# langtech-bsc/quantool

Hardware: AMD Instinct MI355X
Metric: quantized weights/sec (GPTQ int4, Llama-3-8B, 512 calib samples) (higher is better)
Workload: dtype f32

## Files before the change

### include/quantool_amd.h

```cpp
#ifndef QUANTOOL_AMD_H
#define QUANTOOL_AMD_H

#include <stddef.h>
#include <stdint.h>

#ifdef __cplusplus
extern "C" {
#endif

typedef void* qt_stream_t;

enum qt_status {
    QT_OK = 0,
    QT_ERR_INVALID = -1,
    QT_ERR_NOT_PD = -2,
    QT_ERR_WORKSPACE = -3,
    QT_ERR_HIP = -4,
    QT_ERR_UNSUPPORTED = -5
};

enum qt_dtype { QT_F32 = 0, QT_BF16 = 1, QT_F16 = 2 };

int qt_version(void);
const char* qt_last_error(void);
// ... 37 lines not shown
                             const uint8_t* dead, int group_size, int symmetric, int num_bits, float* W_f32, float* scale,
                             float* zp, float* scale_t, float* zp_t, int64_t ld_t, qt_stream_t stream);

size_t qt_gptq_sweep_workspace_bytes(int R, int K, int blocksize);
int qt_gptq_sweep(float* W, int R, int K, const float* U, const float* scale_t, const float* zp_t,
                  int G, const int32_t* g_idx, int blocksize, int num_bits, int8_t* Qt,
                  float* loss, void* workspace, size_t workspace_bytes, qt_stream_t stream);

int qt_gptq_sweep_grouped(float* W, int R, int K, const float* U, int64_t strideU, int n_groups, const int32_t* row_end,
                          const float* scale_t, const float* zp_t, int G, const int32_t* g_idx, int blocksize,
                          int num_bits, int8_t* Qt, float* loss, void* workspace, size_t workspace_bytes,
                          qt_stream_t stream);

int qt_pack_int4(const int8_t* Qt, int R, int K, const int32_t* col_src, int32_t* packed,
                 qt_stream_t stream);

int qt_dequantize(const int8_t* Qt, int R, int K, const int32_t* col_src, const float* scale,
                  const float* zp, int G, const int32_t* g_of_col, void* out, int out_dtype,
                  int64_t ldo, qt_stream_t stream);

size_t qt_awq_weight_mean_workspace_bytes(int R, int K);
int qt_awq_weight_mean_accumulate(const void* W, int w_dtype, int R, int K, int64_t ldw, int group_size,
                                  float* w_sum, void* workspace, size_t workspace_bytes,
                                  qt_stream_t stream);
int qt_awq_scales(const float* x_abs_sum, int64_t n_tokens, const float* w_sum, int64_t n_rows, int K,
                  int n_grid, int duo_scaling, float* scales, qt_stream_t stream);
int qt_symmetrize_lower(float* G, int K, qt_stream_t stream);
size_t qt_awq_loss_workspace_bytes(int R, int K);
int qt_awq_loss(const void* W, int w_dtype, int R, int K, int64_t ldw, const float* s, int group_size,
                int symmetric, int num_bits, const float* Gfull, int64_t n_tokens, int exact, float weight,
                int accumulate, float* loss_out, void* workspace, size_t workspace_bytes, qt_stream_t stream);
size_t qt_awq_losses_workspace_bytes(int R, int K, int n_grid);
int qt_awq_losses(const void* W, int w_dtype, int R, int K, int64_t ldw, const float* scales, int n_grid,
                  int group_size, int symmetric, int num_bits, const float* Gfull, int64_t n_tokens, float weight,
                  int accumulate, float* losses, void* workspace, size_t workspace_bytes, qt_stream_t stream);
int qt_argmin_f32(const float* values, int n, int32_t* index_out, qt_stream_t stream);
int qt_awq_pseudo_quantize(const void* W, int w_dtype, int R, int K, int64_t ldw, const float* s, int group_size,
                           int symmetric, int num_bits, void* out, int64_t ldo, qt_stream_t stream);
int qt_scale_columns(const void* W, int w_dtype, int R, int K, int64_t ldw, const float* s, int divide,
                     void* out, int64_t ldo, qt_stream_t stream);
int qt_rtn_quantize(const void* W, int w_dtype, int R, int K, int64_t ldw, const float* scale,
                    const float* zp, int G, int group_size, int num_bits, int8_t* Qt, qt_stream_t stream);

size_t qt_col_absmax_workspace_bytes(int R, int K);
int qt_col_absmax_accumulate(const void* W, int w_dtype, int R, int K, int64_t ldw, float* wmax,
                             void* workspace, size_t workspace_bytes, qt_stream_t stream);
int qt_smoothquant_scales(const float* cmin, const float* cmax, const float* wmax, int K, float alpha,
                          float* s, qt_stream_t stream);

size_t qt_sgemm_tn_f32_workspace_bytes(int M, int N);
int qt_sgemm_tn_f32(const float* A, int64_t lda, const float* B, int64_t ldb, const float* Cin,
                    int64_t ldcin, float* Cout, int64_t ldcout, int M, int N, int kdim, int skip_zero_k,
                    int mode, int allow_split_k, void* workspace, size_t workspace_bytes, qt_stream_t stream);

int qt_xtx_tile_table_check(int K, int* n_tiles_out, int* chunk_panels_out, int* round_panels_out);

size_t qt_xtx_dot_workspace_bytes(int64_t n_tokens, int K);
int qt_xtx_dot(const void* X, int x_dtype, int64_t n_tokens, int K, int64_t ldx, const float* H, double scale,
               float* out, int accumulate, void* workspace, size_t workspace_bytes, qt_stream_t stream);

size_t qt_gemm3_tn_f32_workspace_bytes(int M, int N, int k);
int qt_gemm3_tn_f32(const float* A, int64_t lda, const float* B, int64_t ldb, float* C, int64_t ldc, int M,
                    int N, int k, int kind, void* workspace, size_t workspace_bytes, qt_stream_t stream);
int qt_gemm3_tn_f32_ex(const float* A, int64_t lda, const float* B, int64_t ldb, float* C, int64_t ldc, int M, int N,
                       int k, int kind, int tri, int tight, int batch, int64_t bsA, int64_t bsB, int64_t bsC,
                       void* workspace, size_t workspace_bytes, qt_stream_t stream);

int qt_gemm3_plan_check(int Tm, int Tn, int c_end, int tri, int* n_items_out, int* n_slabs_out, int* longest_out);
#define QT_I8_MID_MAX_M 128
#define QT_I8_MID_K_UNIT 128
#define QT_I8_RING_K_UNIT 128
#define QT_I8_RING_SLOTS 8
#define QT_I8_RING_LEAD 6
#define QT_I8_RING_W4_K_UNIT 128
#define QT_I8_RING_W4_SLOTS 8
#define QT_I8_RING_W4_LEAD 6
enum qt_weight_format { QT_W_INT8 = 0, QT_W_INT4_PACKED = 1 };
int qt_quantize_tokens_i8(const void* X, int x_dtype, int64_t M, int K, int64_t ldx, const int32_t* col_perm,
                          int symmetric, int8_t* Xq, float* s_x, int32_t* zp_x, qt_stream_t stream);
int qt_gemm_i8(const int8_t* Xq, int64_t M, int K, const void* Wq, int w_format, int N, const float* s_x,
               const int32_t* zp_x, const float* s_w, int G, const int32_t* wsum, const void* bias, void* Y,
               int out_dtype, int64_t ldy, qt_stream_t stream);
int qt_gemm_i8_skinny(const int8_t* Xq, int M, int K, const void* Wq, int w_format, int N, const float* s_x,
                      const int32_t* zp_x, const float* s_w, int G, const int32_t* wsum, const void* bias, void* Y,
                      int out_dtype, int64_t ldy, qt_stream_t stream);
int qt_gemm_i8_ring(const int8_t* Xq, int64_t M, int K, const void* Wq, int w_format, int N, const float* s_x,
                    const int32_t* zp_x, const float* s_w, int G, const int32_t* wsum, const void* bias, void* Y,
                    int out_dtype, int64_t ldy, qt_stream_t stream);
int qt_gemm_i8_ring_w4(const int8_t* Xq, int64_t M, int K, const void* Wq, int w_format, int N, const float* s_x,
                       const int32_t* zp_x, const float* s_w, int G, const int32_t* wsum, const void* bias, void* Y,
                       int out_dtype, int64_t ldy, qt_stream_t stream);
int qt_gemm_i8_mid(const int8_t* Xq, int64_t M, int K, const void* Wq, int w_format, int N, const float* s_x,
                   const int32_t* zp_x, const float* s_w, int G, const int32_t* wsum, const void* bias, void* Y,
                   int out_dtype, int64_t ldy, qt_stream_t stream);

int qt_moe_route(const void* top_k_index, int index_is_int64, int64_t T, int k, int E, int32_t* offsets,
                 int32_t* src_token, int32_t* src_slot, int32_t* row_of, qt_stream_t stream);
int qt_gemm_i8_grouped(const int8_t* Xq, int K, const int32_t* row_idx, int64_t R, const int32_t* offsets, int E,
                       const void* Wq, int w_format, int N, const float* s_x, const int32_t* zp_x, const float* s_w,
                       int G, const int32_t* wsum, void* Y, int out_dtype, int64_t ldy, qt_stream_t stream);
int qt_gemm_i8_skinny_grouped(const int8_t* Xq, int K, const int32_t* row_idx, int64_t R, const int32_t* offsets,
                              int E, const void* Wq, int w_format, int N, const float* s_x, const int32_t* zp_x,
                              const float* s_w, int G, const int32_t* wsum, void* Y, int out_dtype, int64_t ldy,
                              qt_stream_t stream);
int qt_gemm_i8_ring_grouped(const int8_t* Xq, int K, const int32_t* row_idx, int64_t R, const int32_t* offsets, int E,
                            const void* Wq, int w_format, int N, const float* s_x, const int32_t* zp_x,
// ... 24 lines not shown
```

### quantool_amd/csrc/cholesky.hip

```cpp
#include <stdlib.h>
#include <string.h>

#include <map>
#include <tuple>
#include <vector>

#include "common.h"
#include "gemm3_tn.h"
#include "sgemm_tn.h"

namespace {

constexpr int NB = 128;
constexpr int NBO_MAX = 1024;
static int chol_block_env(const char* name) {
    const char* e = getenv(name);
    if (!e) return 0;
    int x = atoi(e) / 128 * 128;
    return x < 128 ? 128 : (x > NBO_MAX ? NBO_MAX : x);
}
struct G3Step {
    int n_items = 0, n_red = 0;
    size_t item_off = 0, red_off = 0;
};
// ... 464 lines not shown
        }
}

__global__ __launch_bounds__(256) void transpose_lower_block_kernel(const float* __restrict__ Y, int64_t ldy, int w,
                                                                    float* __restrict__ XT, int ldx, int64_t bsY,
                                                                    int64_t bsXT) {
    if (blockIdx.z) {
        Y += (size_t)blockIdx.z * bsY;
        XT += (size_t)blockIdx.z * bsXT;
    }
    __shared__ float tile[32][33];
    const int bx = blockIdx.x * 32, by = blockIdx.y * 32;
    const int tx = threadIdx.x & 31, ty = threadIdx.x >> 5;
    for (int r = ty; r < 32; r += 8) {
        const int m = bx + r, k = by + tx;
        tile[r][tx] = (m < w && k < w && k <= m) ? Y[(size_t)m * ldy + k] : 0.0f;
    }
    __syncthreads();
    for (int r = ty; r < 32; r += 8) {
        const int k = by + r, m = bx + tx;
        if (k < w && m < w) XT[(size_t)k * ldx + m] = tile[tx][r];
    }
}

__global__ __launch_bounds__(256) void flat_reverse_lower_to_upper_kernel(float* __restrict__ U, int K, int64_t bsU) {
    U += (size_t)blockIdx.z * bsU;
    const int j = blockIdx.x * blockDim.x + threadIdx.x;
    const int i = blockIdx.y;
    if (j >= K || j < i) return;
    const size_t e = (size_t)i * K + j;
    const size_t pe = (size_t)(K - 1 - i) * K + (K - 1 - j);
    if (i == j) {
        if (e <= pe) {
            const float t = U[e];
            U[e] = U[pe];
            U[pe] = t;
        }
    } else {
        U[e] = U[pe];
        U[pe] = 0.0f;
    }
}

__global__ __launch_bounds__(256) void identity_if_failed_kernel(float* __restrict__ U, int K,
                                                                 const int32_t* __restrict__ info, int64_t bsU) {
    if (info[blockIdx.z] == 0) return;
    U += (size_t)blockIdx.z * bsU;
    for (int i = blockIdx.x; i < K; i += gridDim.x)
        for (int j = threadIdx.x; j < K; j += blockDim.x) U[(size_t)i * K + j] = (i == j) ? 1.0f : 0.0f;
}

}

static size_t chol_problem_ws_bytes(int K, const CholG3Plan* g3) {
    const size_t nb = (K + NB - 1) / NB;
    const size_t split = (size_t)2048 * NB * NB * 4 + (size_t)NBO_MAX * K * 4;
    size_t n = (size_t)NB * K * 4 + (size_t)NBO_MAX * K * 4 + (size_t)NBO_MAX * NBO_MAX * 4 + nb * (NB * NB + RD_STRIDE) * 4 + split + 256;
    if (g3->any) n += 2 * qt_align_up((size_t)3 * K * K * 2, 256) + (size_t)g3->max_slabs * 256 * 256 * 4 + 256;
    return qt_align_up(n, 256);
}

extern "C" size_t qt_cholesky_inverse_upper_batched_workspace_bytes(int K, int n_problems) {
    if (K <= 0 || n_problems <= 0) return 0;
    int nbo_, nbi_;
    const CholG3Plan* g3 = chol_blocks(K, nbo_, nbi_);
    return (size_t)n_problems * chol_problem_ws_bytes(K, g3) + g3->blob_bytes + 512;
}

extern "C" size_t qt_cholesky_inverse_upper_workspace_bytes(int K) {
    return qt_cholesky_inverse_upper_batched_workspace_bytes(K, 1);
}

static int chol_run(float* A, int64_t strideA, int K, float* U, int64_t strideU, int32_t* info, int nprob, void* workspace,
                    size_t workspace_bytes, hipStream_t stream) {
    const size_t need = qt_cholesky_inverse_upper_batched_workspace_bytes(K, nprob);
    if (!workspace || workspace_bytes < need) {
        qt_set_error("qt_cholesky_inverse_upper: workspace %zu < required %zu", workspace_bytes, need);
        return QT_ERR_WORKSPACE;
    }
    const int nblk = (K + NB - 1) / NB;
    char* ws = (char*)qt_align_up((size_t)workspace, 256);
    int NBO, NBI;
    const CholG3Plan* g3 = chol_blocks(K, NBO, NBI);
    const size_t prob_bytes = chol_problem_ws_bytes(K, g3);
    const int64_t sW = (int64_t)(prob_bytes / 4);
    const int64_t sA = nprob > 1 ? strideA : 0, sU = nprob > 1 ? strideU : 0;
    float* T = (float*)ws;
    float* TI = T + (size_t)NB * K;
    float* XT = TI + (size_t)NBO_MAX * K;
    float* Rd = XT + (size_t)NBO_MAX * NBO_MAX;
    float* Dinv = Rd + (size_t)nblk * RD_STRIDE;
    float* split_ws = Dinv + (size_t)nblk * NB * NB;
    const size_t split_ws_bytes = (size_t)2048 * NB * NB * 4 + (size_t)NBO_MAX * K * 4;
    unsigned short *Rpl = nullptr, *Ypl = nullptr;
    float* g3_slabs = nullptr;
    char* g3_tab = nullptr;
    const int64_t plane_stride = (int64_t)K * K;
    if (g3->any) {
        char* q = (char*)qt_align_up((size_t)((char*)split_ws + split_ws_bytes), 256);
        Rpl = (unsigned short*)q;
        q += qt_align_up((size_t)3 * K * K * 2, 256);
        Ypl = (unsigned short*)q;
        q += qt_align_up((size_t)3 * K * K * 2, 256);
        g3_slabs = (float*)q;
        g3_tab = (char*)qt_align_up((size_t)(ws + (size_t)nprob * prob_bytes), 256);
        QT_HIP(hipMemcpyAsync(g3_tab, g3->blob, g3->blob_bytes, hipMemcpyHostToDevice, stream));
    }
    auto g3_row = [&](const G3Step& st, const unsigned short* Bplanes, int col_a0, int col_b0, int M, int N, float* C,
                      int64_t bsC, int mode) -> int {
        G3Args a;
        a.Apl = Rpl;
        a.Bpl = Bplanes;
        a.plane_stride = plane_stride;
        a.ld = K;
        a.rowA0 = a.rowB0 = 0;
        a.colA0 = col_a0;
        a.colB0 = col_b0;
        a.colmax = K;
        a.M = M;
        a.N = N;
        a.C = C;
        a.ldc = K;
        a.mode = mode;
        a.slabs = g3_slabs;
        a.items = (const G3Item*)(g3_tab + st.item_off);
        a.n_items = st.n_items;
        a.red = (const G3Red*)(g3_tab + st.red_off);
        a.n_red = st.n_red;
        a.batch = nprob;
        a.bsApl = a.bsBpl = sW * 2;
        a.bsC = bsC;
        a.bsSlabs = sW;
        return qt_gemm3_launch(a, stream);
    };
    auto sgemm = [&](SgemmArgs& g, int64_t bsA_, int64_t bsB_, int64_t bsC_) -> int {
        g.batch = nprob;
        g.bsA = bsA_;
        g.bsB = bsB_;
        g.bsCin = g.bsCout = bsC_;
        g.bs_split = sW;
        return qt_sgemm_tn(g, stream);
// ... 43 lines not shown
        for (int j0 = J0; j0 < J1; j0 += NB) {
            const int j = j0 / NB, nbj = (K - j0 < NB) ? K - j0 : NB;
            float* Ajj = A + (size_t)j0 * K + j0;
            if (j0 > J0) {
                SgemmArgs g;
                g.A = A + (size_t)J0 * K + j0; g.lda = K;
                g.B = A + (size_t)J0 * K + j0; g.ldb = K;
                g.Cin = Ajj; g.ldcin = K;
                g.Cout = Ajj; g.ldcout = K;
                g.M = nbj; g.N = K - j0; g.kdim = j0 - J0; g.k_mode = SG_K_FULL; g.mode = SG_MODE_SUB;
                int rc = sgemm(g, sA, sA, sA);
                if (rc) return rc;
            }
            hipLaunchKernelGGL(potf2_kernel, dim3(nprob), dim3(POTF2_THREADS), potf2_lds, stream, (const float*)Ajj, (int64_t)K, nbj,
                               Ajj, (int64_t)K, Rd + (size_t)j * RD_STRIDE, info, j0, prio, sA, sW);
            QT_LAUNCH_CHECK();
            const int rest = K - j0 - nbj;
            if (rest > 0) {
                hipLaunchKernelGGL(trsm_rt_kernel, dim3((rest + 127) / 128, nprob), dim3(256), RD_STRIDE * sizeof(float),
                                   stream, (const float*)(Rd + (size_t)j * RD_STRIDE), nbj, (const float*)(Ajj + nbj),
                                   (int64_t)K, Ajj + nbj, (int64_t)K, rest, prio, sW, sA);
                QT_LAUNCH_CHECK();
            }
        }
        const int rem = K - J1;
        if (g3->any) {
            if (rem > 0) {
                int rc = qt_split3_launch(A + (size_t)J0 * K + J0, K, J1 - J0, K - J0, Rpl + (size_t)J0 * K + J0, K,
                                          plane_stride, 0, 0, 0, stream, nprob, sA, sW * 2);
                if (rc) return rc;
            }
        } else if (rem > 0) {
            SgemmArgs g;
            g.A = A + (size_t)J0 * K + J1; g.lda = K;
            g.B = A + (size_t)J0 * K + J1; g.ldb = K;
            g.Cin = A + (size_t)J1 * K + J1; g.ldcin = K;
            g.Cout = A + (size_t)J1 * K + J1; g.ldcout = K;
            g.M = rem; g.N = rem; g.kdim = J1 - J0; g.k_mode = SG_K_FULL; g.mode = SG_MODE_SUB;
            g.upper_only = 1;
            int rc = sgemm(g, sA, sA, sA);
            if (rc) return rc;
        }
    }
    {
        const char* e = getenv("QT_CHOL_TRINV");
        if (e && strcmp(e, "div") == 0)
            hipLaunchKernelGGL(trinv_batched_kernel, dim3(nblk, nprob), dim3(NB), inv_lds, stream, (const float*)Rd, K, Dinv, Y,
                               (int64_t)K, sW, sY);
        else
            hipLaunchKernelGGL(trinv_mfma_kernel, dim3(nblk, nprob), dim3(256), RD_STRIDE * sizeof(float), stream,
                               (const float*)Rd, K, Dinv, Y, (int64_t)K, sW, sY);
    }
    QT_LAUNCH_CHECK();
    for (int I0 = 0, Ib = 0; I0 < K; I0 += NBI, ++Ib) {
        const int I1 = (K - I0 < NBI) ? K : I0 + NBI;
        const int Wi = I1 - I0;
        for (int i0 = I0 + NB; i0 < I1; i0 += NB) {
            const int i = i0 / NB, nbi = (K - i0 < NB) ? K - i0 : NB;
            SgemmArgs g;
            g.A = A + (size_t)I0 * K + i0; g.lda = K;
            g.B = Y + (size_t)I0 * K + I0; g.ldb = K;
            g.Cin = nullptr; g.ldcin = 0;
            g.Cout = T; g.ldcout = K;
            g.M = nbi; g.N = i0 - I0; g.kdim = i0 - I0; g.k_mode = SG_K_FROM_N0; g.mode = SG_MODE_SET;
            int rc = sgemm(g, sA, sY, sW);
            if (rc) return rc;
            SgemmArgs t;
            t.A = Dinv + (size_t)i * NB * NB; t.lda = NB;
            t.B = T; t.ldb = K;
            t.Cin = nullptr; t.ldcin = 0;
            t.Cout = Y + (size_t)i0 * K + I0; t.ldcout = K;
            t.M = nbi; t.N = i0 - I0; t.kdim = nbi; t.k_mode = SG_K_FULL; t.mode = SG_MODE_NEG;
            rc = sgemm(t, sW, sW, sY);
            if (rc) return rc;
        }
        auto split_row = [&]() -> int {
            if (!g3->any || I1 >= K) return QT_OK;
            return qt_split3_launch(Y + (size_t)I0 * K, K, Wi, I1, Ypl + (size_t)I0 * K, K, plane_stride, 1, I0, 0, stream,
                                    nprob, sY, sW * 2);
        };
        if (I0 == 0) {
            int rc0 = split_row();
            if (rc0) return rc0;
            continue;
        }
        int rc;
        if (g3->any && g3->inv[Ib].n_items > 0) {
            rc = g3_row(g3->inv[Ib], Ypl, I0, 0, Wi, I0, TI, sW, G3_SET);
        } else {
            SgemmArgs g;
            g.A = A + I0; g.lda = K;
            g.B = Y; g.ldb = K;
            g.Cin = nullptr; g.ldcin = 0;
            g.Cout = TI; g.ldcout = K;
            g.M = Wi; g.N = I0; g.kdim = I0; g.k_mode = SG_K_FROM_N0; g.mode = SG_MODE_SET;
            g.split_ws = split_ws; g.split_ws_bytes = split_ws_bytes;
            rc = sgemm(g, sA, sY, sW);
        }
        if (rc) return rc;
        hipLaunchKernelGGL(transpose_lower_block_kernel, dim3((Wi + 31) / 32, (Wi + 31) / 32, nprob), dim3(256), 0, stream,
                           (const float*)(Y + (size_t)I0 * K + I0), (int64_t)K, Wi, XT, NBO_MAX, sY, sW);
        QT_LAUNCH_CHECK();
        SgemmArgs t;
        t.A = XT; t.lda = NBO_MAX;
        t.B = TI; t.ldb = K;
        t.Cin = nullptr; t.ldcin = 0;
        t.Cout = Y + (size_t)I0 * K; t.ldcout = K;
        t.M = Wi; t.N = I0; t.kdim = Wi; t.k_mode = SG_K_FULL; t.mode = SG_MODE_NEG;
        rc = sgemm(t, sW, sW, sY);
        if (rc) return rc;
// ... 27 lines not shown
```

### quantool_amd/csrc/sgemm_tn.h

```cpp
#pragma once
#include "common.h"

enum { SG_MODE_SUB = 0, SG_MODE_SET = 1, SG_MODE_NEG = 2 };
enum { SG_K_FULL = 0, SG_K_FROM_N0 = 1 };
constexpr int SG_MAX_GROUPS = 16;
constexpr int SG_MAX_BATCH = 16;

struct SgemmArgs {
    const float* A; int64_t lda;
    const float* B; int64_t ldb;
    const float* Cin; int64_t ldcin;
    float* Cout; int64_t ldcout;
    int M, N, kdim;
    int k_mode;
    int mode;
    float* split_ws = nullptr;
    size_t split_ws_bytes = 0;
    int chain_len = 0;
    int upper_only = 0;
    int batch = 1;
    int64_t bsA = 0, bsB = 0, bsCin = 0, bsCout = 0;
    int64_t bs_split = 0;
    int n_groups = 0;
    int64_t group_bsB = 0;
    int group_m_end[SG_MAX_GROUPS] = {};
    int k_chunk = 0;
    int n_splits = 1;
    int fast_interior = 1;
};

int qt_sgemm_tn(const SgemmArgs& a, hipStream_t stream);

int qt_splitk_reduce(const float* slabs, int splits, int M, int N, const float* Cin, int64_t ldcin, float* Cout,
                     int64_t ldcout, int mode, hipStream_t stream, int batch = 1, int64_t bs_slabs = 0, int64_t bs_cin = 0,
                     int64_t bs_cout = 0);
```

### quantool_amd/csrc/sgemm_tn.hip

```cpp
#include <stdlib.h>

#include <type_traits>

#include "ring_pipe.h"
#include "sgemm_tn.h"

namespace {

constexpr int BK = 16;

#ifndef QT_SGEMM_PD
#define QT_SGEMM_PD 2
#endif

template <int N, class F>
__device__ __forceinline__ void sg_static_for(F&& f) {
    if constexpr (N > 0) {
        sg_static_for<N - 1>(f);
        f(std::integral_constant<int, N - 1>{});
    }
}

template <int BM, int BN, int MODE, bool CHAIN = false, int NWAVE = 4>
__global__ __launch_bounds__(64 * NWAVE) __attribute__((amdgpu_waves_per_eu(NWAVE == 8 ? 4 : 2))) void sgemm_tn_kernel(const SgemmArgs p) {
    constexpr int NT = 64 * NWAVE;
    constexpr int WGM = NWAVE == 8 ? 4 : 2, WGN = 2;
    constexpr int WM = BM / (32 * WGM), WN = BN / (32 * WGN);
    constexpr int A4 = BK * BM / 4 / NT;
    constexpr int B4 = BK * BN / 4 / NT;
    static_assert(A4 >= 1 && B4 >= 1, "tile too small for the workgroup");
    __shared__ __attribute__((aligned(16))) float As[2][BK][BM];
    __shared__ __attribute__((aligned(16))) float Bs[2][BK][BN];

    const int tid = threadIdx.x, lane = tid & 63, wave = tid >> 6;
    const int wave_m = wave >> 1, wave_n = wave & 1;
    const int m0 = blockIdx.y * BM, n0 = blockIdx.x * BN;
    if (p.upper_only && m0 >= n0 + BN) return;
    const float* Ap = p.A;
    const float* Bp = p.B;
    const float* Cinp = p.Cin;
    float* Coutp = p.Cout;
    int zsplit = blockIdx.z;
    if (p.batch > 1) {
        const int b = zsplit / p.n_splits;
        zsplit -= b * p.n_splits;
        Ap += (size_t)b * p.bsA;
        Bp += (size_t)b * p.bsB;
        if (Cinp) Cinp += (size_t)b * p.bsCin;
        Coutp += (size_t)b * p.bsCout;
    }
    if (p.n_groups > 0) {
        int g = 0;
        while (g + 1 < p.n_groups && m0 >= p.group_m_end[g]) ++g;
        Bp += (size_t)g * p.group_bsB;
    }
    const bool tile_inside = p.fast_interior && m0 + BM <= p.M && n0 + BN <= p.N;

    int k_begin = 0;
    if (p.k_mode == SG_K_FROM_N0) k_begin = n0 / BK * BK;
    int k_end = p.kdim;
    if (p.k_chunk > 0) {
        const int lo = zsplit * p.k_chunk, hi = lo + p.k_chunk;
        k_begin = k_begin > lo ? k_begin : lo;
        k_end = k_end < hi ? k_end : hi;
        Coutp += (size_t)zsplit * (size_t)p.M * (size_t)p.N;
    }

    const bool a_vec = (p.lda % 4 == 0) && (((uintptr_t)Ap & 15) == 0);
    const bool b_vec = (p.ldb % 4 == 0) && (((uintptr_t)Bp & 15) == 0);

    constexpr int PD = (BM == 64 && BN == 64 && !CHAIN) ? QT_SGEMM_PD : 1;
    static_assert(PD == 1 || PD % 2 == 0, "the LDS buffer of a step is s & 1: the unrolled ring must be even");
    f32x4 ra[PD][A4], rb[PD][B4];

    const bool interior = p.fast_interior && a_vec && b_vec && m0 + BM <= p.M && n0 + BN <= p.N;
    auto gload_fast = [&](int k0, auto slot_c) {
        constexpr int slot = decltype(slot_c)::value;
#pragma unroll
        for (int r = 0; r < A4; ++r) {
            const int idx = tid + NT * r;
            ra[slot][r] = *(const f32x4*)(Ap + (size_t)(k0 + idx / (BM / 4)) * p.lda + m0 + (idx % (BM / 4)) * 4);
        }
#pragma unroll
        for (int r = 0; r < B4; ++r) {
            const int idx = tid + NT * r;
            rb[slot][r] = *(const f32x4*)(Bp + (size_t)(k0 + idx / (BN / 4)) * p.ldb + n0 + (idx % (BN / 4)) * 4);
        }
    };
    auto gload = [&](int k0, auto slot_c) {
        constexpr int slot = decltype(slot_c)::value;
        if (interior && k0 + BK <= k_end) {
            gload_fast(k0, slot_c);
            return;
        }
#pragma unroll
// ... 334 lines not shown
        batch_prev = 32;
        if (it + 1 < my_tiles) {
            size_t oa, ob;
            tile_origin(it + 1, m0, n0, oa, ob, c_off_in, c_off_out);
        }
    }
}

__global__ __launch_bounds__(256) void splitk_reduce_kernel(const float* __restrict__ slabs, int splits, int M,
                                                            int N, const float* __restrict__ Cin, int64_t ldcin,
                                                            float* __restrict__ Cout, int64_t ldcout, int mode,
                                                            int64_t bs_slabs, int64_t bs_cin, int64_t bs_cout) {
    const int col = (blockIdx.x * blockDim.x + threadIdx.x) * 4;
    const int row = blockIdx.y;
    if (col >= N) return;
    if (blockIdx.z) {
        slabs += (size_t)blockIdx.z * bs_slabs;
        if (Cin) Cin += (size_t)blockIdx.z * bs_cin;
        Cout += (size_t)blockIdx.z * bs_cout;
    }
    const size_t mn = (size_t)M * N;
    if (col + 3 < N && (N & 3) == 0) {
        f32x4 s = {0.f, 0.f, 0.f, 0.f};
        const float* src = slabs + (size_t)row * N + col;
        int z = 0;
        for (; z + 8 <= splits; z += 8) {
            f32x4 v[8];
#pragma unroll
            for (int u = 0; u < 8; ++u) v[u] = *(const f32x4*)(src + (size_t)(z + u) * mn);
#pragma unroll
            for (int u = 0; u < 8; ++u) s += v[u];
        }
        for (; z < splits; ++z) s += *(const f32x4*)(src + (size_t)z * mn);
#pragma unroll
        for (int e = 0; e < 4; ++e) {
            float v = s[e];
            if (mode == SG_MODE_SUB) v = Cin[(size_t)row * ldcin + col + e] - v;
            if (mode == SG_MODE_NEG) v = -v;
            Cout[(size_t)row * ldcout + col + e] = v;
        }
    } else {
        for (int e = 0; e < 4 && col + e < N; ++e) {
            float v = 0.f;
            for (int z = 0; z < splits; ++z) v += slabs[z * mn + (size_t)row * N + col + e];
            if (mode == SG_MODE_SUB) v = Cin[(size_t)row * ldcin + col + e] - v;
            if (mode == SG_MODE_NEG) v = -v;
            Cout[(size_t)row * ldcout + col + e] = v;
        }
    }
}

template <int BM, int BN>
int launch(const SgemmArgs& a, hipStream_t stream, int splits = 1) {
    dim3 grid((a.N + BN - 1) / BN, (a.M + BM - 1) / BM, splits * (a.batch > 1 ? a.batch : 1));
    static const bool sub8 = [] {
        const char* e = getenv("QT_SGEMM_SUB_WAVES");
        return !(e && atoi(e) == 4);
    }();
    switch (a.mode) {
        case SG_MODE_SUB:
            if constexpr (BM == 128 && BN == 128) {
                if (sub8) {
                    if (a.chain_len > 0)
                        hipLaunchKernelGGL((sgemm_tn_kernel<BM, BN, SG_MODE_SUB, true, 8>), grid, dim3(512), 0, stream, a);
                    else
                        hipLaunchKernelGGL((sgemm_tn_kernel<BM, BN, SG_MODE_SUB, false, 8>), grid, dim3(512), 0, stream, a);
                    break;
                }
            }
            if (a.chain_len > 0)
                hipLaunchKernelGGL((sgemm_tn_kernel<BM, BN, SG_MODE_SUB, true>), grid, dim3(256), 0, stream, a);
            else
                hipLaunchKernelGGL((sgemm_tn_kernel<BM, BN, SG_MODE_SUB>), grid, dim3(256), 0, stream, a);
            break;
        case SG_MODE_SET:
            hipLaunchKernelGGL((sgemm_tn_kernel<BM, BN, SG_MODE_SET>), grid, dim3(256), 0, stream, a);
            break;
        default:
            hipLaunchKernelGGL((sgemm_tn_kernel<BM, BN, SG_MODE_NEG>), grid, dim3(256), 0, stream, a);
            break;
    }
    QT_LAUNCH_CHECK();
    return QT_OK;
}

}

int qt_splitk_reduce(const float* slabs, int splits, int M, int N, const float* Cin, int64_t ldcin, float* Cout,
                     int64_t ldcout, int mode, hipStream_t stream, int batch, int64_t bs_slabs, int64_t bs_cin,
                     int64_t bs_cout) {
    hipLaunchKernelGGL(splitk_reduce_kernel, dim3((N / 4 + 255) / 256 + 1, M, batch > 1 ? batch : 1), dim3(256), 0, stream,
                       slabs, splits, M, N, Cin, ldcin, Cout, ldcout, mode, bs_slabs, bs_cin, bs_cout);
    QT_LAUNCH_CHECK();
    return QT_OK;
}

int qt_sgemm_tn(const SgemmArgs& a_, hipStream_t stream) {
    if (a_.M <= 0 || a_.N <= 0) return QT_OK;
    QT_CHECK_ARG(a_.batch >= 1 && a_.batch <= SG_MAX_BATCH && a_.n_groups >= 0 && a_.n_groups <= SG_MAX_GROUPS &&
                     !(a_.batch > 1 && a_.n_groups > 0),
                 "qt_sgemm_tn: batch %d / row groups %d unsupported", a_.batch, a_.n_groups);
    for (int g = 0; g < a_.n_groups; ++g)
        QT_CHECK_ARG((a_.group_m_end[g] % 128 == 0 || g == a_.n_groups - 1) && (g == 0 || a_.group_m_end[g] >= a_.group_m_end[g - 1]),
                     "qt_sgemm_tn: row group %d ends at %d (boundaries must be ascending multiples of 128)", g, a_.group_m_end[g]);
    static const int fast_interior = [] {
        const char* e = getenv("QT_SGEMM_INTERIOR");
        return (e && atoi(e) == 0) ? 0 : 1;
    }();
    SgemmArgs a = a_;
    a.fast_interior = fast_interior;
    const long t128 = (long)((a.M + 127) / 128) * ((a.N + 127) / 128);
    if (a.split_ws && t128 < 384 && a.kdim >= 512) {
        static const int target_wgs = [] {
            const char* e = getenv("QT_SGEMM_SPLIT_TARGET");
            const int v = e ? atoi(e) : 256;
            return v < 256 ? 256 : v;
        }();
        static const int min_chunk = [] {
            const char* e = getenv("QT_SGEMM_SPLIT_MIN_CHUNK");
            const int v = e ? atoi(e) : 128;
            return v < 64 ? 64 : v;
        }();
        int splits = (int)(target_wgs / t128);
        if (splits > 32) splits = 32;
        if (splits < 1) splits = 1;
        int chunk = (a.kdim + splits - 1) / splits;
        chunk = (chunk + 63) / 64 * 64;
        if (chunk < min_chunk) chunk = min_chunk;
        splits = (a.kdim + chunk - 1) / chunk;
        const size_t need = (size_t)splits * a.M * a.N * sizeof(float);
        if (splits >= 2 && need <= a.split_ws_bytes && (a.batch <= 1 || (size_t)a.bs_split * sizeof(float) >= need)) {
            SgemmArgs part = a;
            part.Cin = nullptr;
            part.ldcin = 0;
            part.Cout = a.split_ws;
            part.ldcout = a.N;
            part.bsCin = 0;
            part.bsCout = a.bs_split;
            part.mode = SG_MODE_SET;
            part.k_chunk = chunk;
            part.n_splits = splits;
            const int rc = launch<128, 128>(part, stream, splits);
            if (rc) return rc;
            return qt_splitk_reduce(a.split_ws, splits, a.M, a.N, a.Cin, a.ldcin, a.Cout, a.ldcout, a.mode, stream, a.batch,
                                    a.bs_split, a.bsCin, a.bsCout);
        }
    }
    const char* ring_env = getenv("QT_SGEMM_RING");
    const int use_ring = (ring_env && atoi(ring_env) == 0) ? 0 : 1;
    const char* ring_min_env = getenv("QT_SGEMM_RING_MIN_TILES");
    const int ring_min_tiles = ring_min_env ? atoi(ring_min_env) : 32;
    if (use_ring && a.mode == SG_MODE_SUB && a.k_mode == SG_K_FULL && a.k_chunk == 0 && a.kdim >= 4 * RBK &&
        a.kdim % (2 * RBK) == 0 && (a.chain_len == 0 || (a.chain_len % (2 * RBK) == 0 && a.kdim % a.chain_len == 0)) &&
        a.kdim % RBK == 0 && (a.chain_len == 0 || a.chain_len % RBK == 0) && a.M % RBM == 0 && a.N % RBN == 0 &&
        (size_t)40 * (size_t)(a.ldcin > a.ldcout ? a.ldcin : a.ldcout) * 4 < ((size_t)1 << 31) && a.lda % 4 == 0 &&
        a.ldb % 4 == 0 && (((uintptr_t)a.A | (uintptr_t)a.B) & 15) == 0 &&
        (size_t)RBK * (size_t)(a.lda > a.ldb ? a.lda : a.ldb) * 4 < ((size_t)1 << 32) && (!a.upper_only || a.M == a.N)) {
        RingArgs r;
        r.A = a.A; r.lda = a.lda; r.B = a.B; r.ldb = a.ldb;
        r.Cin = a.Cin; r.ldcin = a.ldcin; r.Cout = a.Cout; r.ldcout = a.ldcout;
        r.M = a.M; r.N = a.N; r.kdim = a.kdim;
        r.chain_len = a.chain_len > 0 ? a.chain_len : a.kdim;
        const int tm = (a.M + RBM - 1) / RBM, tn = (a.N + RBN - 1) / RBN;
        r.tiles_n = tn;
        r.upper_only = a.upper_only;
        r.n_tiles = a.upper_only ? tn * (tn + 1) / 2 : tm * tn;
        r.batch = a.batch > 1 ? a.batch : 1;
        r.bsA = a.bsA; r.bsB = a.bsB; r.bsCin = a.bsCin; r.bsCout = a.bsCout;
        r.n_groups = a.n_groups;
        r.group_bsB = a.group_bsB;
        for (int g = 0; g < SG_MAX_GROUPS; ++g) r.group_m_end[g] = a.group_m_end[g];
        if (r.n_tiles >= ring_min_tiles) {
            const int all = r.n_tiles * r.batch;
            const int grid = all >= 2 * 256 ? 2 * 256 : all;
            hipLaunchKernelGGL(sgemm_ring_kernel, dim3(grid), dim3(512), 0, stream, r);
            QT_LAUNCH_CHECK();
            return QT_OK;
        }
    }
    if (t128 >= 384) return launch<128, 128>(a, stream);
    return launch<64, 64>(a, stream);
}

extern "C" size_t qt_sgemm_tn_f32_workspace_bytes(int M, int N) {
    if (M <= 0 || N <= 0) return 0;
    return (size_t)32 * M * N * 4 + 256;
}

extern "C" int qt_sgemm_tn_f32(const float* A, int64_t lda, const float* B, int64_t ldb, const float* Cin,
                               int64_t ldcin, float* Cout, int64_t ldcout, int M, int N, int kdim, int skip_zero_k,
                               int mode, int allow_split_k, void* workspace, size_t workspace_bytes,
                               qt_stream_t stream_) {
    hipStream_t stream = (hipStream_t)stream_;
    QT_CHECK_ARG(A && B && Cout && M > 0 && N > 0 && kdim >= 0, "qt_sgemm_tn_f32: bad arguments");
    QT_CHECK_ARG(mode == SG_MODE_SUB || mode == SG_MODE_SET || mode == SG_MODE_NEG, "qt_sgemm_tn_f32: mode %d", mode);
    QT_CHECK_ARG(mode != SG_MODE_SUB || Cin, "qt_sgemm_tn_f32: MODE_SUB needs Cin");
    SgemmArgs g;
    g.A = A; g.lda = lda;
    g.B = B; g.ldb = ldb;
    g.Cin = Cin; g.ldcin = ldcin;
    g.Cout = Cout; g.ldcout = ldcout;
    g.M = M; g.N = N; g.kdim = kdim;
    g.k_mode = skip_zero_k ? SG_K_FROM_N0 : SG_K_FULL;
    g.mode = mode;
    if (allow_split_k) {
        const size_t need = qt_sgemm_tn_f32_workspace_bytes(M, N);
        if (!workspace || workspace_bytes < need) {
            qt_set_error("qt_sgemm_tn_f32: workspace %zu < required %zu", workspace_bytes, need);
            return QT_ERR_WORKSPACE;
        }
        g.split_ws = (float*)qt_align_up((size_t)workspace, 256);
        g.split_ws_bytes = workspace_bytes - 256;
    }
    return qt_sgemm_tn(g, stream);
}
```

### quantool_amd/hip/_lib.py

```python
from __future__ import annotations

import ctypes
from ctypes import c_char_p, c_double, c_float, c_int, c_int32, c_int64, c_size_t, c_void_p
from pathlib import Path

_PKG = Path(__file__).resolve().parent.parent
LIB_PATH = _PKG / "lib" / "libquantool_hip.so"

QT_OK = 0
QT_ERR_INVALID = -1
QT_ERR_NOT_PD = -2
QT_ERR_WORKSPACE = -3
QT_ERR_HIP = -4
QT_ERR_UNSUPPORTED = -5

QT_F32, QT_BF16, QT_F16 = 0, 1, 2
QT_W_INT8, QT_W_INT4_PACKED = 0, 1

SIGNATURES = {
    "qt_version": (c_int, []),
    "qt_last_error": (c_char_p, []),
    "qt_xtx_workspace_bytes": (c_size_t, [c_int64, c_int]),
    "qt_xtx_accumulate": (c_int, [c_void_p, c_int, c_int64, c_int, c_int64, c_void_p, c_void_p, c_size_t, c_void_p]),
    "qt_xtx_accumulate_f32_workspace_bytes": (c_size_t, [c_int64, c_int]),
# ... 8 lines not shown
    "qt_argsort_desc": (c_int, [c_void_p, c_int, c_void_p, c_void_p, c_void_p]),
    "qt_cholesky_inverse_upper_workspace_bytes": (c_size_t, [c_int]),
    "qt_cholesky_inverse_upper": (c_int, [c_void_p, c_int, c_void_p, c_void_p, c_void_p, c_size_t, c_void_p]),
    "qt_cholesky_inverse_upper_batched_workspace_bytes": (c_size_t, [c_int, c_int]),
    "qt_cholesky_inverse_upper_batched": (c_int, [c_void_p, c_int64, c_int, c_void_p, c_int64, c_void_p, c_int, c_void_p,
                                                  c_size_t, c_void_p]),
    "qt_group_minmax_qparams": (c_int, [c_void_p, c_int, c_int, c_int, c_int64, c_int, c_int, c_int, c_void_p,
                                        c_void_p, c_void_p, c_void_p, c_void_p]),
    "qt_weight_gather_f32": (c_int, [c_void_p, c_int, c_int, c_int, c_int64, c_void_p, c_void_p, c_void_p,
                                     c_void_p]),
    "qt_weight_gather_qparams": (c_int, [c_void_p, c_int, c_int, c_int, c_int64, c_void_p, c_void_p, c_int, c_int, c_int,
                                         c_void_p, c_void_p, c_void_p, c_void_p, c_void_p, c_int64, c_void_p]),
    "qt_gptq_sweep_workspace_bytes": (c_size_t, [c_int, c_int, c_int]),
    "qt_gptq_sweep": (c_int, [c_void_p, c_int, c_int, c_void_p, c_void_p, c_void_p, c_int, c_void_p, c_int, c_int,
                              c_void_p, c_void_p, c_void_p, c_size_t, c_void_p]),
    "qt_gptq_sweep_grouped": (c_int, [c_void_p, c_int, c_int, c_void_p, c_int64, c_int, c_void_p, c_void_p, c_void_p, c_int,
                                      c_void_p, c_int, c_int, c_void_p, c_void_p, c_void_p, c_size_t, c_void_p]),
    "qt_pack_int4": (c_int, [c_void_p, c_int, c_int, c_void_p, c_void_p, c_void_p]),
    "qt_awq_weight_mean_workspace_bytes": (c_size_t, [c_int, c_int]),
    "qt_awq_weight_mean_accumulate": (c_int, [c_void_p, c_int, c_int, c_int, c_int64, c_int, c_void_p, c_void_p,
                                              c_size_t, c_void_p]),
    "qt_awq_scales": (c_int, [c_void_p, c_int64, c_void_p, c_int64, c_int, c_int, c_int, c_void_p, c_void_p]),
    "qt_symmetrize_lower": (c_int, [c_void_p, c_int, c_void_p]),
    "qt_awq_loss_workspace_bytes": (c_size_t, [c_int, c_int]),
    "qt_awq_loss": (c_int, [c_void_p, c_int, c_int, c_int, c_int64, c_void_p, c_int, c_int, c_int, c_void_p, c_int64,
                            c_int, c_float, c_int, c_void_p, c_void_p, c_size_t, c_void_p]),
    "qt_awq_losses_workspace_bytes": (c_size_t, [c_int, c_int, c_int]),
    "qt_awq_losses": (c_int, [c_void_p, c_int, c_int, c_int, c_int64, c_void_p, c_int, c_int, c_int, c_int, c_void_p,
                              c_int64, c_float, c_int, c_void_p, c_void_p, c_size_t, c_void_p]),
    "qt_argmin_f32": (c_int, [c_void_p, c_int, c_void_p, c_void_p]),
    "qt_awq_pseudo_quantize": (c_int, [c_void_p, c_int, c_int, c_int, c_int64, c_void_p, c_int, c_int, c_int, c_void_p,
                                       c_int64, c_void_p]),
    "qt_scale_columns": (c_int, [c_void_p, c_int, c_int, c_int, c_int64, c_void_p, c_int, c_void_p, c_int64,
                                 c_void_p]),
    "qt_rtn_quantize": (c_int, [c_void_p, c_int, c_int, c_int, c_int64, c_void_p, c_void_p, c_int, c_int, c_int,
                                c_void_p, c_void_p]),
    "qt_col_absmax_workspace_bytes": (c_size_t, [c_int, c_int]),
    "qt_col_absmax_accumulate": (c_int, [c_void_p, c_int, c_int, c_int, c_int64, c_void_p, c_void_p, c_size_t,
                                         c_void_p]),
    "qt_smoothquant_scales": (c_int, [c_void_p, c_void_p, c_void_p, c_int, c_float, c_void_p, c_void_p]),
    "qt_xtx_dot_workspace_bytes": (c_size_t, [c_int64, c_int]),
    "qt_xtx_dot": (c_int, [c_void_p, c_int, c_int64, c_int, c_int64, c_void_p, c_double, c_void_p, c_int, c_void_p,
                           c_size_t, c_void_p]),
    "qt_gemm3_plan_check": (c_int, [c_int, c_int, c_int, c_int, c_void_p, c_void_p, c_void_p]),
    "qt_xtx_tile_table_check": (c_int, [c_int, c_void_p, c_void_p, c_void_p]),
    "qt_gemm3_tn_f32_workspace_bytes": (c_size_t, [c_int, c_int, c_int]),
    "qt_gemm3_tn_f32": (c_int, [c_void_p, c_int64, c_void_p, c_int64, c_void_p, c_int64, c_int, c_int, c_int, c_int,
                                c_void_p, c_size_t, c_void_p]),
    "qt_gemm3_tn_f32_ex": (c_int, [c_void_p, c_int64, c_void_p, c_int64, c_void_p, c_int64, c_int, c_int, c_int, c_int,
                                   c_int, c_int, c_int, c_int64, c_int64, c_int64, c_void_p, c_size_t, c_void_p]),
    "qt_sgemm_tn_f32_workspace_bytes": (c_size_t, [c_int, c_int]),
    "qt_sgemm_tn_f32": (c_int, [c_void_p, c_int64, c_void_p, c_int64, c_void_p, c_int64, c_void_p, c_int64, c_int,
                                c_int, c_int, c_int, c_int, c_int, c_void_p, c_size_t, c_void_p]),
    "qt_profile_enable": (c_int, [c_int]),
    "qt_profile_read": (c_int, [c_int, c_void_p, c_void_p]),
    "qt_dequantize": (c_int, [c_void_p, c_int, c_int, c_void_p, c_void_p, c_void_p, c_int, c_void_p, c_void_p,
                              c_int, c_int64, c_void_p]),
    "qt_quantize_tokens_i8": (c_int, [c_void_p, c_int, c_int64, c_int, c_int64, c_void_p, c_int, c_void_p, c_void_p,
                                      c_void_p, c_void_p]),
    "qt_gemm_i8": (c_int, [c_void_p, c_int64, c_int, c_void_p, c_int, c_int, c_void_p, c_void_p, c_void_p, c_int,
                           c_void_p, c_void_p, c_void_p, c_int, c_int64, c_void_p]),
    "qt_gemm_i8_skinny": (c_int, [c_void_p, c_int, c_int, c_void_p, c_int, c_int, c_void_p, c_void_p, c_void_p, c_int,
                                  c_void_p, c_void_p, c_void_p, c_int, c_int64, c_void_p]),
    "qt_gemm_i8_ring": (c_int, [c_void_p, c_int64, c_int, c_void_p, c_int, c_int, c_void_p, c_void_p, c_void_p, c_int,
                                c_void_p, c_void_p, c_void_p, c_int, c_int64, c_void_p]),
    "qt_gemm_i8_ring_w4": (c_int, [c_void_p, c_int64, c_int, c_void_p, c_int, c_int, c_void_p, c_void_p, c_void_p,
                                   c_int, c_void_p, c_void_p, c_void_p, c_int, c_int64, c_void_p]),
    "qt_gemm_i8_mid": (c_int, [c_void_p, c_int64, c_int, c_void_p, c_int, c_int, c_void_p, c_void_p, c_void_p, c_int,
                               c_void_p, c_void_p, c_void_p, c_int, c_int64, c_void_p]),
    "qt_gemm_i8_skinny_grouped": (c_int, [c_void_p, c_int, c_void_p, c_int64, c_void_p, c_int, c_void_p, c_int, c_int,
                                          c_void_p, c_void_p, c_void_p, c_int, c_void_p, c_void_p, c_int, c_int64,
                                          c_void_p]),
    "qt_moe_route": (c_int, [c_void_p, c_int, c_int64, c_int, c_int, c_void_p, c_void_p, c_void_p, c_void_p,
                             c_void_p]),
    "qt_gemm_i8_grouped": (c_int, [c_void_p, c_int, c_void_p, c_int64, c_void_p, c_int, c_void_p, c_int, c_int,
                                   c_void_p, c_void_p, c_void_p, c_int, c_void_p, c_void_p, c_int, c_int64, c_void_p]),
    "qt_gemm_i8_ring_grouped": (c_int, [c_void_p, c_int, c_void_p, c_int64, c_void_p, c_int, c_void_p, c_int, c_int,
                                        c_void_p, c_void_p, c_void_p, c_int, c_void_p, c_void_p, c_int, c_int64,
                                        c_int64, c_void_p]),
    "qt_moe_combine": (c_int, [c_void_p, c_int, c_int, c_int64, c_void_p, c_void_p, c_int64, c_int, c_void_p,
                               c_void_p]),
    "qt_dequantize_weight": (c_int, [c_void_p, c_int, c_int, c_int, c_void_p, c_int, c_void_p, c_void_p, c_void_p,
                                     c_int, c_int64, c_void_p]),
    "qt_gemm_wq_skinny": (c_int, [c_void_p, c_int, c_int, c_int, c_int64, c_void_p, c_int, c_int, c_void_p, c_int,
                                  c_void_p, c_void_p, c_void_p, c_void_p, c_int64, c_void_p]),
    "qt_gemm_wq_grouped": (c_int, [c_void_p, c_int, c_int, c_int64, c_void_p, c_int64, c_void_p, c_int, c_void_p,
                                   c_int, c_int, c_void_p, c_int, c_void_p, c_void_p, c_void_p, c_int64, c_void_p]),
}

_lib = None


class HipBackendError(RuntimeError):

    def __init__(self, fn: str, status: int, message: str):
        super().__init__(f"{fn} failed with status {status}: {message}")
        self.status = status


def load() -> ctypes.CDLL:
    global _lib
    if _lib is not None:
        return _lib
    if not LIB_PATH.exists():
        raise ImportError(
            f"quantool_amd HIP library not found at {LIB_PATH}. Build it with "
# ... 19 lines not shown
```

### quantool_amd/hip/ops.py

```python
from __future__ import annotations

import logging
import os
from typing import Optional

import torch

from . import _lib
from ._lib import QT_BF16, QT_F16, QT_F32, check, load

_WS_CACHE: dict = {}


def _stream() -> int:
    return torch.cuda.current_stream().cuda_stream


def _ptr(t: Optional[torch.Tensor]) -> Optional[int]:
    return None if t is None else t.data_ptr()


def _dtype_code(t: torch.Tensor) -> int:
    if t.dtype == torch.float32:
        return QT_F32
# ... 1046 lines not shown
    return out


def gemm3_tn(A: torch.Tensor, B: torch.Tensor, C: torch.Tensor, kind: int = 0):
    lib = load()
    _req(A, torch.float32, "A", 2)
    _req(B, torch.float32, "B", 2)
    _req(C, torch.float32, "C", 2)
    k, M = A.shape
    k2, N = B.shape
    assert k == k2 and A.stride(1) == 1 and B.stride(1) == 1 and C.stride(1) == 1 and tuple(C.shape) == (M, N)
    ws = workspace(lib.qt_gemm3_tn_f32_workspace_bytes(M, N, k), A.device, "gemm3")
    check("qt_gemm3_tn_f32", lib.qt_gemm3_tn_f32(A.data_ptr(), A.stride(0), B.data_ptr(), B.stride(0), C.data_ptr(),
                                                 C.stride(0), M, N, k, kind, ws.data_ptr(), ws.numel(), _stream()))
    return C


def gemm3_tn_ex(A: torch.Tensor, B: torch.Tensor, C: torch.Tensor, kind: int = 0, tri: bool = False, tight: bool = False):
    lib = load()
    if A.dim() == 2:
        A, B, C3 = A[None], B[None], C[None]
    else:
        C3 = C
    _req(A, torch.float32, "A", 3)
    _req(B, torch.float32, "B", 3)
    _req(C3, torch.float32, "C", 3)
    n, k, M = A.shape
    n2, k2, N = B.shape
    assert n == n2 and k == k2 and tuple(C3.shape) == (n, M, N)
    assert A.is_contiguous() and B.is_contiguous() and C3.is_contiguous()
    ws = workspace(n * lib.qt_gemm3_tn_f32_workspace_bytes(M, N, k), A.device, "gemm3")
    check("qt_gemm3_tn_f32_ex", lib.qt_gemm3_tn_f32_ex(A.data_ptr(), M, B.data_ptr(), N, C3.data_ptr(), N, M, N, k, kind,
                                                       int(tri), int(tight), n, k * M, k * N, M * N, ws.data_ptr(),
                                                       ws.numel(), _stream()))
    return C


def sgemm_tn(A: torch.Tensor, B: torch.Tensor, Cin: Optional[torch.Tensor] = None, mode: int = 1,
             skip_zero_k: bool = False, allow_split_k: bool = False, out: Optional[torch.Tensor] = None):
    lib = load()
    _req(A, torch.float32, "A", 2)
    _req(B, torch.float32, "B", 2)
    k, M = A.shape
    k2, N = B.shape
    assert k == k2 and A.stride(1) == 1 and B.stride(1) == 1
    if out is None:
        out = torch.empty((M, N), dtype=torch.float32, device=A.device)
    ws = workspace(lib.qt_sgemm_tn_f32_workspace_bytes(M, N) if allow_split_k else 1, A.device, "sgemm")
    check("qt_sgemm_tn_f32", lib.qt_sgemm_tn_f32(
        A.data_ptr(), A.stride(0), B.data_ptr(), B.stride(0), _ptr(Cin), Cin.stride(0) if Cin is not None else 0,
        out.data_ptr(), out.stride(0), M, N, k, int(skip_zero_k), mode, int(allow_split_k),
        ws.data_ptr() if allow_split_k else None, ws.numel() if allow_split_k else 0, _stream()))
    return out
```

Baseline: 3.003 billion.

## Batch diagonal-block triangular inverse updates across outer blocks via second sgemm batch dim

Adds a second batch dimension to the sgemm kernel and uses it in the Cholesky inverse. The within-block Y updates for all full NBI-wide diagonal blocks are now issued as one batched launch per NB step, where before they were done block by block in a loop. This cuts the kernel launch count and gives each launch more blocks to fill the GPU. The T scratch buffer grows to hold one panel per outer block, the ring path is disabled for the batched case, and an env var restores the old per-row path.

```diff
diff --git a/include/quantool_amd.h b/include/quantool_amd.h
--- a/include/quantool_amd.h
+++ b/include/quantool_amd.h
@@ -113,6 +113,10 @@
 int qt_sgemm_tn_f32(const float* A, int64_t lda, const float* B, int64_t ldb, const float* Cin,
                     int64_t ldcin, float* Cout, int64_t ldcout, int M, int N, int kdim, int skip_zero_k,
                     int mode, int allow_split_k, void* workspace, size_t workspace_bytes, qt_stream_t stream);
+int qt_sgemm_tn_f32_batched(const float* A, int64_t lda, int64_t bsA, int64_t bs2A, const float* B, int64_t ldb,
+                            int64_t bsB, int64_t bs2B, const float* Cin, int64_t ldcin, int64_t bsCin, int64_t bs2Cin,
+                            float* Cout, int64_t ldcout, int64_t bsCout, int64_t bs2Cout, int M, int N, int kdim,
+                            int skip_zero_k, int mode, int batch, int batch2, qt_stream_t stream);
 
 int qt_xtx_tile_table_check(int K, int* n_tiles_out, int* chunk_panels_out, int* round_panels_out);
 
diff --git a/quantool_amd/csrc/cholesky.hip b/quantool_amd/csrc/cholesky.hip
--- a/quantool_amd/csrc/cholesky.hip
+++ b/quantool_amd/csrc/cholesky.hip
@@ -540,10 +540,12 @@
 
 }
 
-static size_t chol_problem_ws_bytes(int K, const CholG3Plan* g3) {
+static size_t chol_t_floats(int K, int NBI) { return (size_t)((K + NBI - 1) / NBI) * NB * NBI; }
+
+static size_t chol_problem_ws_bytes(int K, int NBI, const CholG3Plan* g3) {
     const size_t nb = (K + NB - 1) / NB;
     const size_t split = (size_t)2048 * NB * NB * 4 + (size_t)NBO_MAX * K * 4;
-    size_t n = (size_t)NB * K * 4 + (size_t)NBO_MAX * K * 4 + (size_t)NBO_MAX * NBO_MAX * 4 + nb * (NB * NB + RD_STRIDE) * 4 + split + 256;
+    size_t n = chol_t_floats(K, NBI) * 4 + (size_t)NBO_MAX * K * 4 + (size_t)NBO_MAX * NBO_MAX * 4 + nb * (NB * NB + RD_STRIDE) * 4 + split + 256;
     if (g3->any) n += 2 * qt_align_up((size_t)3 * K * K * 2, 256) + (size_t)g3->max_slabs * 256 * 256 * 4 + 256;
     return qt_align_up(n, 256);
 }
@@ -552,7 +554,7 @@
     if (K <= 0 || n_problems <= 0) return 0;
     int nbo_, nbi_;
     const CholG3Plan* g3 = chol_blocks(K, nbo_, nbi_);
-    return (size_t)n_problems * chol_problem_ws_bytes(K, g3) + g3->blob_bytes + 512;
+    return (size_t)n_problems * chol_problem_ws_bytes(K, nbi_, g3) + g3->blob_bytes + 512;
 }
 
 extern "C" size_t qt_cholesky_inverse_upper_workspace_bytes(int K) {
@@ -570,11 +572,11 @@
     char* ws = (char*)qt_align_up((size_t)workspace, 256);
     int NBO, NBI;
     const CholG3Plan* g3 = chol_blocks(K, NBO, NBI);
-    const size_t prob_bytes = chol_problem_ws_bytes(K, g3);
+    const size_t prob_bytes = chol_problem_ws_bytes(K, NBI, g3);
     const int64_t sW = (int64_t)(prob_bytes / 4);
     const int64_t sA = nprob > 1 ? strideA : 0, sU = nprob > 1 ? strideU : 0;
     float* T = (float*)ws;
-    float* TI = T + (size_t)NB * K;
+    float* TI = T + chol_t_floats(K, NBI);
     float* XT = TI + (size_t)NBO_MAX * K;
     float* Rd = XT + (size_t)NBO_MAX * NBO_MAX;
     float* Dinv = Rd + (size_t)nblk * RD_STRIDE;
@@ -724,10 +726,38 @@
                                (const float*)Rd, K, Dinv, Y, (int64_t)K, sW, sY);
     }
     QT_LAUNCH_CHECK();
+    const char* yii_env = getenv("QT_CHOL_YII");
+    const bool yii_rows = yii_env && strcmp(yii_env, "rows") == 0;
+    const int n_full = K / NBI;
+    if (!yii_rows && n_full > 0) {
+        const int64_t sRow = (int64_t)NBI * K + NBI;
+        const int64_t sT = (int64_t)NB * NBI;
+        for (int s = 1; s < NBI / NB; ++s) {
+            const int w = s * NB;
+            SgemmArgs g;
+            g.A = A + w; g.lda = K;
+            g.B = Y; g.ldb = K;
+            g.Cin = nullptr; g.ldcin = 0;
+            g.Cout = T; g.ldcout = NBI;
+            g.M = NB; g.N = w; g.kdim = w; g.k_mode = SG_K_FROM_N0; g.mode = SG_MODE_SET;
+            g.batch2 = n_full; g.bs2A = sRow; g.bs2B = sRow; g.bs2Cout = sT;
+            int rc = sgemm(g, sA, sY, sW);
+            if (rc) return rc;
+            SgemmArgs t;
+            t.A = Dinv + (size_t)s * NB * NB; t.lda = NB;
+            t.B = T; t.ldb = NBI;
+            t.Cin = nullptr; t.ldcin = 0;
+            t.Cout = Y + (size_t)w * K; t.ldcout = K;
+            t.M = NB; t.N = w; t.kdim = NB; t.k_mode = SG_K_FULL; t.mode = SG_MODE_NEG;
+            t.batch2 = n_full; t.bs2A = (int64_t)NBI * NB; t.bs2B = sT; t.bs2Cout = sRow;
+            rc = sgemm(t, sW, sW, sY);
+            if (rc) return rc;
+        }
+    }
     for (int I0 = 0, Ib = 0; I0 < K; I0 += NBI, ++Ib) {
         const int I1 = (K - I0 < NBI) ? K : I0 + NBI;
         const int Wi = I1 - I0;
-        for (int i0 = I0 + NB; i0 < I1; i0 += NB) {
+        for (int i0 = I0 + NB; i0 < I1 && (yii_rows || Wi < NBI); i0 += NB) {
             const int i = i0 / NB, nbi = (K - i0 < NB) ? K - i0 : NB;
             SgemmArgs g;
             g.A = A + (size_t)I0 * K + i0; g.lda = K;
diff --git a/quantool_amd/csrc/sgemm_tn.h b/quantool_amd/csrc/sgemm_tn.h
--- a/quantool_amd/csrc/sgemm_tn.h
+++ b/quantool_amd/csrc/sgemm_tn.h
@@ -21,6 +21,8 @@
     int batch = 1;
     int64_t bsA = 0, bsB = 0, bsCin = 0, bsCout = 0;
     int64_t bs_split = 0;
+    int batch2 = 1;
+    int64_t bs2A = 0, bs2B = 0, bs2Cin = 0, bs2Cout = 0;
     int n_groups = 0;
     int64_t group_bsB = 0;
     int group_m_end[SG_MAX_GROUPS] = {};
diff --git a/quantool_amd/csrc/sgemm_tn.hip b/quantool_amd/csrc/sgemm_tn.hip
--- a/quantool_amd/csrc/sgemm_tn.hip
+++ b/quantool_amd/csrc/sgemm_tn.hip
@@ -41,6 +41,15 @@
     const float* Cinp = p.Cin;
     float* Coutp = p.Cout;
     int zsplit = blockIdx.z;
+    if (p.batch2 > 1) {
+        const int per = (p.batch > 1 ? p.batch : 1) * p.n_splits;
+        const int b2 = zsplit / per;
+        zsplit -= b2 * per;
+        Ap += (size_t)b2 * p.bs2A;
+        Bp += (size_t)b2 * p.bs2B;
+        if (Cinp) Cinp += (size_t)b2 * p.bs2Cin;
+        Coutp += (size_t)b2 * p.bs2Cout;
+    }
     if (p.batch > 1) {
         const int b = zsplit / p.n_splits;
         zsplit -= b * p.n_splits;
@@ -481,7 +490,7 @@
 
 template <int BM, int BN>
 int launch(const SgemmArgs& a, hipStream_t stream, int splits = 1) {
-    dim3 grid((a.N + BN - 1) / BN, (a.M + BM - 1) / BM, splits * (a.batch > 1 ? a.batch : 1));
+    dim3 grid((a.N + BN - 1) / BN, (a.M + BM - 1) / BM, splits * (a.batch > 1 ? a.batch : 1) * (a.batch2 > 1 ? a.batch2 : 1));
     static const bool sub8 = [] {
         const char* e = getenv("QT_SGEMM_SUB_WAVES");
         return !(e && atoi(e) == 4);
@@ -529,6 +538,11 @@
     QT_CHECK_ARG(a_.batch >= 1 && a_.batch <= SG_MAX_BATCH && a_.n_groups >= 0 && a_.n_groups <= SG_MAX_GROUPS &&
                      !(a_.batch > 1 && a_.n_groups > 0),
                  "qt_sgemm_tn: batch %d / row groups %d unsupported", a_.batch, a_.n_groups);
+    constexpr int SG_GRID_Z_MAX = 65535;
+    QT_CHECK_ARG(a_.batch2 >= 1 && (a_.batch2 == 1 || (a_.split_ws == nullptr && a_.n_groups == 0 &&
+                                                       (long)a_.batch2 * a_.batch <= SG_GRID_Z_MAX)),
+                 "qt_sgemm_tn: outer batch %d unsupported (x batch %d <= %d, no split-K workspace, no row groups)", a_.batch2,
+                 a_.batch, SG_GRID_Z_MAX);
     for (int g = 0; g < a_.n_groups; ++g)
         QT_CHECK_ARG((a_.group_m_end[g] % 128 == 0 || g == a_.n_groups - 1) && (g == 0 || a_.group_m_end[g] >= a_.group_m_end[g - 1]),
                      "qt_sgemm_tn: row group %d ends at %d (boundaries must be ascending multiples of 128)", g, a_.group_m_end[g]);
@@ -579,7 +593,7 @@
     const int use_ring = (ring_env && atoi(ring_env) == 0) ? 0 : 1;
     const char* ring_min_env = getenv("QT_SGEMM_RING_MIN_TILES");
     const int ring_min_tiles = ring_min_env ? atoi(ring_min_env) : 32;
-    if (use_ring && a.mode == SG_MODE_SUB && a.k_mode == SG_K_FULL && a.k_chunk == 0 && a.kdim >= 4 * RBK &&
+    if (use_ring && a.batch2 <= 1 && a.mode == SG_MODE_SUB && a.k_mode == SG_K_FULL && a.k_chunk == 0 && a.kdim >= 4 * RBK &&
         a.kdim % (2 * RBK) == 0 && (a.chain_len == 0 || (a.chain_len % (2 * RBK) == 0 && a.kdim % a.chain_len == 0)) &&
         a.kdim % RBK == 0 && (a.chain_len == 0 || a.chain_len % RBK == 0) && a.M % RBM == 0 && a.N % RBN == 0 &&
         (size_t)40 * (size_t)(a.ldcin > a.ldcout ? a.ldcin : a.ldcout) * 4 < ((size_t)1 << 31) && a.lda % 4 == 0 &&
@@ -643,3 +657,29 @@
     }
     return qt_sgemm_tn(g, stream);
 }
+
+extern "C" int qt_sgemm_tn_f32_batched(const float* A, int64_t lda, int64_t bsA, int64_t bs2A, const float* B, int64_t ldb,
+                                       int64_t bsB, int64_t bs2B, const float* Cin, int64_t ldcin, int64_t bsCin,
+                                       int64_t bs2Cin, float* Cout, int64_t ldcout, int64_t bsCout, int64_t bs2Cout, int M,
+                                       int N, int kdim, int skip_zero_k, int mode, int batch, int batch2,
+                                       qt_stream_t stream_) {
+    hipStream_t stream = (hipStream_t)stream_;
+    QT_CHECK_ARG(A && B && Cout && M > 0 && N > 0 && kdim >= 0, "qt_sgemm_tn_f32_batched: bad arguments");
+    QT_CHECK_ARG(mode == SG_MODE_SUB || mode == SG_MODE_SET || mode == SG_MODE_NEG, "qt_sgemm_tn_f32_batched: mode %d", mode);
+    QT_CHECK_ARG(mode != SG_MODE_SUB || Cin, "qt_sgemm_tn_f32_batched: MODE_SUB needs Cin");
+    QT_CHECK_ARG(batch >= 1 && batch <= SG_MAX_BATCH && batch2 >= 1, "qt_sgemm_tn_f32_batched: batch %d (1..%d), batch2 %d",
+                 batch, SG_MAX_BATCH, batch2);
+    SgemmArgs g;
+    g.A = A; g.lda = lda;
+    g.B = B; g.ldb = ldb;
+    g.Cin = Cin; g.ldcin = ldcin;
+    g.Cout = Cout; g.ldcout = ldcout;
+    g.M = M; g.N = N; g.kdim = kdim;
+    g.k_mode = skip_zero_k ? SG_K_FROM_N0 : SG_K_FULL;
+    g.mode = mode;
+    g.batch = batch;
+    g.bsA = bsA; g.bsB = bsB; g.bsCin = bsCin; g.bsCout = bsCout;
+    g.batch2 = batch2;
+    g.bs2A = bs2A; g.bs2B = bs2B; g.bs2Cin = bs2Cin; g.bs2Cout = bs2Cout;
+    return qt_sgemm_tn(g, stream);
+}
diff --git a/quantool_amd/hip/_lib.py b/quantool_amd/hip/_lib.py
--- a/quantool_amd/hip/_lib.py
+++ b/quantool_amd/hip/_lib.py
@@ -84,6 +84,9 @@
     "qt_sgemm_tn_f32_workspace_bytes": (c_size_t, [c_int, c_int]),
     "qt_sgemm_tn_f32": (c_int, [c_void_p, c_int64, c_void_p, c_int64, c_void_p, c_int64, c_void_p, c_int64, c_int,
                                 c_int, c_int, c_int, c_int, c_int, c_void_p, c_size_t, c_void_p]),
+    "qt_sgemm_tn_f32_batched": (c_int, [c_void_p, c_int64, c_int64, c_int64, c_void_p, c_int64, c_int64, c_int64, c_void_p,
+                                        c_int64, c_int64, c_int64, c_void_p, c_int64, c_int64, c_int64, c_int, c_int,
+                                        c_int, c_int, c_int, c_int, c_int, c_void_p]),
     "qt_profile_enable": (c_int, [c_int]),
     "qt_profile_read": (c_int, [c_int, c_void_p, c_void_p]),
     "qt_dequantize": (c_int, [c_void_p, c_int, c_int, c_void_p, c_void_p, c_void_p, c_int, c_void_p, c_void_p,
diff --git a/quantool_amd/hip/ops.py b/quantool_amd/hip/ops.py
--- a/quantool_amd/hip/ops.py
+++ b/quantool_amd/hip/ops.py
@@ -1122,3 +1122,23 @@
         out.data_ptr(), out.stride(0), M, N, k, int(skip_zero_k), mode, int(allow_split_k),
         ws.data_ptr() if allow_split_k else None, ws.numel() if allow_split_k else 0, _stream()))
     return out
+
+
+def sgemm_tn_batched(A: torch.Tensor, B: torch.Tensor, Cin: Optional[torch.Tensor] = None, mode: int = 1,
+                     skip_zero_k: bool = False, out: Optional[torch.Tensor] = None):
+    lib = load()
+    _req(A, torch.float32, "A", 4)
+    _req(B, torch.float32, "B", 4)
+    n2, n1, k, M = A.shape
+    N = B.shape[3]
+    assert tuple(B.shape[:3]) == (n2, n1, k) and A.stride(3) == 1 and B.stride(3) == 1
+    if out is None:
+        out = torch.empty((n2, n1, M, N), dtype=torch.float32, device=A.device)
+    assert tuple(out.shape) == (n2, n1, M, N) and out.stride(3) == 1
+    assert Cin is None or (tuple(Cin.shape) == (n2, n1, M, N) and Cin.stride(3) == 1)
+    cs = Cin.stride() if Cin is not None else (0, 0, 0, 1)
+    check("qt_sgemm_tn_f32_batched", lib.qt_sgemm_tn_f32_batched(
+        A.data_ptr(), A.stride(2), A.stride(1), A.stride(0), B.data_ptr(), B.stride(2), B.stride(1), B.stride(0),
+        _ptr(Cin), cs[2], cs[1], cs[0], out.data_ptr(), out.stride(2), out.stride(1), out.stride(0), M, N, k,
+        int(skip_zero_k), mode, n1, n2, _stream()))
+    return out
```

Measured after the change: 3.017 billion (median of 6 runs). About the same (+0.5%).
